# LittleWat/multichannel-semseg-with-uda

Hardware: AMD Instinct MI355X
Metric: RGB-D img/s (6x480x640) MCD train step, drn_d_38 (higher is better)
Workload: dtype f32 (operands split 2-way into scaled fp16, 3 cross terms on the fp16 MFMA pipe, fp32 accumulate)

## Files before the change

### multichannel-semseg-with-uda_amd/csrc/conv_gemm_split.hip

```cpp
#include <cstdlib>
#include <type_traits>

#include "conv_split_params.h"
#include "options.h"

namespace {


template <class P, int WM, int WN, int WAVES_M, int WAVES_N, bool DGRAD, bool PRESPLIT>
__global__ __launch_bounds__(256, 2) void conv_gemm_split_kernel(ConvSplitParams p) {
  constexpr int BM = 32 * WM * WAVES_M;
  constexpr int BN = 32 * WN * WAVES_N;
  constexpr int NT = 256;
  static_assert(WAVES_M * WAVES_N == 4, "4 waves per workgroup");
  constexpr int B_ITEMS = BN * 2 / NT;
  constexpr int NP = P::NP;
  constexpr int NQ = 2 * NP;
  typedef typename P::frag frag;
  constexpr int A_CHUNKS = NQ * BM;
  constexpr int A_ITERS = (A_CHUNKS + NT - 1) / NT;
  constexpr bool A_EXACT = (A_CHUNKS % NT) == 0;
  constexpr bool A_DMA = A_EXACT;
  constexpr int A_ITERS_DMA = ((2 * P::NPU * BM) % NT == 0) ? (2 * P::NPU * BM) / NT : A_ITERS;
  constexpr int A_BYTES = NQ * BM * 16, B_BYTES = NQ * BN * 16;

  constexpr bool B_DMA = PRESPLIT && A_DMA && (B_ITEMS == 1 || (BM == 128 && BN == 256));
  constexpr int NSTAGE = (B_DMA && 3 * (A_BYTES + B_BYTES) <= 80 * 1024) ? 3 : 2;

  __shared__ __attribute__((aligned(16))) unsigned char smem[NSTAGE * (A_BYTES + B_BYTES)];
  unsigned char* As = smem;
  unsigned char* Bs = smem + NSTAGE * A_BYTES;

  const int t = threadIdx.x;
  const int lane = t & 63;
  const int wave = t >> 6;
  const int wm = wave / WAVES_N;
  const int wn = wave % WAVES_N;
  const int l31 = lane & 31, lh = lane >> 5;

  const int m_tiles = p.Mp / BM;
  const bool SUB = DGRAD && p.sub != 0;
  const int n_tiles = SUB ? p.cls_tile0[4] : p.tile_n1;
  const int tile_n0 = SUB ? 0 : p.tile_n0;
  const int per_xcd = (n_tiles - tile_n0 + 7) >> 3;
  const int xcd = blockIdx.x & 7;
  const int slot = blockIdx.x >> 3;
  const int tile_m = slot % m_tiles;
  const int tile_n = tile_n0 + xcd * per_xcd + slot / m_tiles;
  if (tile_n >= n_tiles) return;

  const int bj = t % BN;
  const int bh0 = __builtin_amdgcn_readfirstlane(t / BN);
  const int HWd = p.Hd * p.Wd;
  const int HWs = p.Hs * p.Ws;
  int cls = 0;
  const bool ILV = SUB && p.sub == 2;
  const bool ROW = SUB && p.sub == 3;
  if (SUB) cls = ILV ? (tile_n & 3) : (tile_n >= p.cls_tile0[1]) + (tile_n >= p.cls_tile0[2]) + (tile_n >= p.cls_tile0[3]);
  const int ry = ROW ? cls : cls >> 1, rx = cls & 1;
  const int Hc = SUB ? (p.Hd - ry + 1) >> 1 : p.Hd;
  const int Wc = SUB && !ROW ? (p.Wd - rx + 1) >> 1 : p.Wd;
  const int HWc = Hc * Wc;
  const int Pc = SUB ? p.N * HWc : p.P;
  const int ltile = SUB ? (ILV ? tile_n >> 2 : tile_n - p.cls_tile0[cls]) : tile_n;
  const int pix = ltile * BN + bj;
  const bool pv = pix < Pc;
  int pn = 0, py = 0, px = 0, yc = 0, xc = 0;
  if (pv) {
    pn = pix / HWc;
    const int rem = pix - pn * HWc;
    yc = rem / Wc;
    xc = rem - yc * Wc;
    py = SUB ? 2 * yc + ry : yc;
    px = SUB && !ROW ? 2 * xc + rx : xc;
  }
  unsigned cls_taps = 0;
  if (SUB) {
    for (int q = 0; q < p.KH * p.KW; ++q) {
      const int qy = q / p.KW, qx = q - qy * p.KW;
      if ((((ry + p.pad - qy * p.dil) | (ROW ? 0 : rx + p.pad - qx * p.dil)) & 1) == 0) cls_taps |= 1u << q;
    }
  }
  constexpr unsigned OOB = 0x80000000u;
  constexpr unsigned UNIT = PRESPLIT ? 16u : 4u;
  const __amdgpu_buffer_rsrc_t src_rs = PRESPLIT ? __builtin_amdgcn_make_buffer_rsrc((void*)p.src_cb, 0, p.cb_bytes, 0x00020000)
                                                 : __builtin_amdgcn_make_buffer_rsrc((void*)p.src, 0, p.src_bytes, 0x00020000);
  __amdgpu_buffer_rsrc_t cb_rs[NP];
#pragma unroll
  for (int pc = 0; pc < NP; ++pc)
    cb_rs[pc] = __builtin_amdgcn_make_buffer_rsrc((void*)((const char*)p.src_cb + pc * p.cb_piece_stride), 0, PRESPLIT ? p.cb_bytes : 0, 0x00020000);
  const __amdgpu_buffer_rsrc_t wp_rs = __builtin_amdgcn_make_buffer_rsrc((void*)p.wp, 0, p.wp_bytes, 0x00020000);
  const int C8 = p.Cs >> 3;
  const float inv_src_scale = 1.f / operand_scale<P>(p.src_bound);
  const unsigned pix_base = PRESPLIT ? (unsigned)pn * (unsigned)C8 * (unsigned)HWs : (unsigned)pn * (unsigned)p.Cs * (unsigned)HWs;
  const bool ragged = p.Kp != p.Cs;
  const int taps = p.KH * p.KW;

  int l_tap = 0, l_c0 = 0, l_ky = 0, l_kx = 0, l_kstep = 0;
  unsigned l_voff = OOB;
  auto tap_geom = [&]() {
    bool ok;
    int off;
    if (!DGRAD) {
      const int sy = py * p.stride + l_ky * p.dil - p.pad;
      const int sx = px * p.stride + l_kx * p.dil - p.pad;
      ok = pv && sy >= 0 && sy < p.Hs && sx >= 0 && sx < p.Ws;
      off = sy * p.Ws + sx;
    } else {
      const int ty = py + p.pad - l_ky * p.dil;
      const int tx = px + p.pad - l_kx * p.dil;
      ok = pv && ty >= 0 && tx >= 0;
      int sy = ty, sx = tx;
// ... 112 lines not shown
    const int a_soff = (l_kstep * NQ * p.Mp + tile_m * BM) * 16;
    if (A_DMA) return;
#pragma unroll
    for (int i = 0; i < A_ITERS; ++i) {
      const auto q = __builtin_amdgcn_raw_buffer_load_b128(wp_rs, a_voff[i], a_soff, 0);
      areg[SET][i][0] = __uint_as_float(q[0]);
      areg[SET][i][1] = __uint_as_float(q[1]);
      areg[SET][i][2] = __uint_as_float(q[2]);
      areg[SET][i][3] = __uint_as_float(q[3]);
    }
  };
  auto dma_weights = [&](int buf) {
    const int a_soff = (l_kstep * NQ * p.Mp + tile_m * BM) * 16;
    unsigned char* adst = As + buf * A_BYTES + wave * 64 * 16;
#if defined(__HIP_DEVICE_COMPILE__)
#pragma unroll
    for (int i = 0; i < A_ITERS_DMA; ++i)
      __builtin_amdgcn_raw_ptr_buffer_load_lds(wp_rs, (__attribute__((address_space(3))) void*)(adst + i * NT * 16), 16, a_voff[i], a_soff, 0, 0);
#else
    (void)a_soff;
    (void)adst;
#endif
  };
  auto store_lds = [&](int buf, auto set_c) {
    constexpr int SET = decltype(set_c)::value;
    unsigned char* bdst = Bs + buf * B_BYTES;
#pragma unroll
    for (int it = 0; it < B_ITEMS; ++it) {
      const int h = (B_ITEMS == 1) ? bh0 : it;
      if constexpr (PRESPLIT) {
#pragma unroll
        for (int pc = 0; pc < NP; ++pc) *reinterpret_cast<f32x4*>(bdst + ((pc * 2 + h) * BN + bj) * 16) = bsplit[SET][it][pc];
        continue;
      }
      if constexpr (!PRESPLIT) {
        frag pieces[NP];
        split_frag<P>(breg[SET][it], inv_src_scale, pieces);
#pragma unroll
        for (int pc = 0; pc < NP; ++pc) *reinterpret_cast<frag*>(bdst + ((pc * 2 + h) * BN + bj) * 16) = pieces[pc];
      }
    }
    if (!A_DMA) {
      unsigned char* adst = As + buf * A_BYTES;
#pragma unroll
      for (int i = 0; i < A_ITERS; ++i) {
        const int id = t + i * NT;
        if (A_EXACT || id < A_CHUNKS) *reinterpret_cast<f32x4*>(adst + id * 16) = areg[SET][i];
      }
    }
  };

  f32x16 acc[WM][WN];
#pragma unroll
  for (int i = 0; i < WM; ++i)
#pragma unroll
    for (int j = 0; j < WN; ++j)
#pragma unroll
      for (int r = 0; r < 16; ++r) acc[i][j][r] = 0.f;

  const int nsteps = (SUB ? __builtin_popcount(cls_taps) : taps) * (p.Kp / 16);
  using S0 = std::integral_constant<int, 0>;
  using S1 = std::integral_constant<int, 1>;
  int l_dma_kstep = l_kstep;
  int dma_tap = l_tap, dma_c0 = 0;
  auto dma_b = [&](int buf) {
    const int wave_px = __builtin_amdgcn_readfirstlane(bj - lane);
#pragma unroll
    for (int it = 0; it < B_ITEMS; ++it) {
      const int h = (B_ITEMS == 1) ? bh0 : it;
      const int grp = (l_c0 >> 3) + h;
      unsigned char* bdst = Bs + buf * B_BYTES + (h * BN + wave_px) * 16;
#if defined(__HIP_DEVICE_COMPILE__)
#pragma unroll
      for (int pc = 0; pc < P::NPU; ++pc) {
        const int soff = grp < C8 ? grp * HWs * 16 : 0x7FFFFFFF;
        __builtin_amdgcn_raw_ptr_buffer_load_lds(cb_rs[pc], (__attribute__((address_space(3))) void*)(bdst + pc * 2 * BN * 16), 16, l_voff, soff, 0, 0);
      }
#else
      (void)grp;
      (void)bdst;
#endif
    }
  };
  constexpr int DMA_PER_STEP = A_ITERS_DMA + P::NPU * B_ITEMS;
  if constexpr (B_DMA) {
    if (nsteps > 0) {
      dma_weights(0);
      dma_b(0);
    }
    if (NSTAGE == 3 && nsteps > 1) {
      advance();
      dma_weights(1);
      dma_b(1);
      asm volatile("s_waitcnt vmcnt(%0) lgkmcnt(0)\n\ts_barrier" ::"n"(DMA_PER_STEP) : "memory");
    } else {
      asm volatile("s_waitcnt vmcnt(0) lgkmcnt(0)\n\ts_barrier" ::: "memory");
    }
  } else {
    if (nsteps > 0) {
      if (A_DMA) dma_weights(0);
      load_regs(S0{});
      store_lds(0, S0{});
      if (nsteps > 1) {
        advance();
        load_regs(S1{});
      }
    }
    __syncthreads();
  }

  frag fa[NP][WM], fb[NP][WN];
  auto read_frags = [&](int cur) {
    const unsigned char* a_base = As + cur * A_BYTES + (lh * BM + wm * (32 * WM) + l31) * 16;
    const unsigned char* b_base = Bs + cur * B_BYTES + (lh * BN + wn * (32 * WN) + l31) * 16;
#pragma unroll
    for (int pc = 0; pc < NP; ++pc) {
#pragma unroll
      for (int i = 0; i < WM; ++i) fa[pc][i] = *reinterpret_cast<const frag*>(a_base + (pc * 2 * BM + i * 32) * 16);
#pragma unroll
      for (int j = 0; j < WN; ++j) fb[pc][j] = *reinterpret_cast<const frag*>(b_base + (pc * 2 * BN + j * 32) * 16);
    }
  };
  auto mfma_frags = [&]() {
#if defined(MCD_SETPRIO)
    __builtin_amdgcn_s_setprio(1);
#endif
#if defined(MCD_MFMA_TILE_MAJOR)
#pragma unroll
    for (int i = 0; i < WM; ++i)
#pragma unroll
      for (int j = 0; j < WN; ++j)
#pragma unroll
        for (int tm = 0; tm < P::NTERMS; ++tm) acc[i][j] = P::mfma(fa[P::TA[tm]][i], fb[P::TB[tm]][j], acc[i][j]);
#else
#pragma unroll
    for (int tm = 0; tm < P::NTERMS; ++tm)
#pragma unroll
      for (int i = 0; i < WM; ++i)
#pragma unroll
        for (int j = 0; j < WN; ++j) acc[i][j] = P::mfma(fa[P::TA[tm]][i], fb[P::TB[tm]][j], acc[i][j]);
#endif
#if defined(MCD_SETPRIO)
    __builtin_amdgcn_s_setprio(0);
#endif
  };
  auto mfma_step = [&](int cur) {
    read_frags(cur);
    mfma_frags();
  };
  auto k_step = [&](int s, auto cur_c, auto steady_c) {
    constexpr int CUR = decltype(cur_c)::value;
    constexpr bool STEADY = decltype(steady_c)::value;
    using SAME = std::integral_constant<int, CUR>;
    using OTHER = std::integral_constant<int, CUR ^ 1>;
    if (A_DMA && (STEADY || s + 1 < nsteps)) {
      if (SUB) {
        const unsigned rest = cls_taps & ~((2u << dma_tap) - 1u);
        if (rest) {
          dma_tap = __builtin_ctz(rest);
        } else {
          dma_tap = __builtin_ctz(cls_taps);
          dma_c0 += 16;
        }
        l_dma_kstep = (dma_c0 >> 4) * taps + dma_tap;
      } else {
        ++l_dma_kstep;
// ... 18 lines not shown
    if (STEADY || s + 1 < nsteps) store_lds(CUR ^ 1, OTHER{});
    if constexpr (A_DMA) {
      constexpr int AHEAD = (PRESPLIT ? NP : 8) * B_ITEMS;
      if (STEADY || s + 2 < nsteps)
        asm volatile("s_waitcnt vmcnt(%0) lgkmcnt(0)\n\ts_barrier" ::"n"(AHEAD) : "memory");
      else
        asm volatile("s_waitcnt vmcnt(0) lgkmcnt(0)\n\ts_barrier" ::: "memory");
    } else {
      __syncthreads();
    }
  };
  using YES = std::integral_constant<bool, true>;
  using NO = std::integral_constant<bool, false>;
  if constexpr (B_DMA && NSTAGE == 3) {
    int cur = 0, nxt2 = 2;
    for (int s = 0; s < nsteps; ++s) {
      const bool more2 = s + 2 < nsteps;
#if defined(MCD_ABLATE) && (MCD_ABLATE & 4)
      if (s == 0)
#endif
      read_frags(cur);
      __builtin_amdgcn_sched_barrier(0);
      if (more2) {
        advance();
#if !defined(MCD_ABLATE) || !(MCD_ABLATE & 1)
        dma_weights(nxt2);
#endif
#if defined(MCD_ABLATE) && (MCD_ABLATE & 64)
        if (l_tap == 0) dma_b(nxt2);
#elif !defined(MCD_ABLATE) || !(MCD_ABLATE & 2)
        dma_b(nxt2);
#endif
      }
      __builtin_amdgcn_sched_barrier(0);
#if !defined(MCD_ABLATE) || !(MCD_ABLATE & 8)
      mfma_frags();
#endif
#if defined(MCD_ABLATE) && (MCD_ABLATE & 16)
      asm volatile("s_waitcnt lgkmcnt(0)\n\ts_barrier" ::: "memory");
#elif defined(MCD_ABLATE) && (MCD_ABLATE & 32)
      if (more2)
        asm volatile("s_waitcnt vmcnt(%0) lgkmcnt(0)" ::"n"(DMA_PER_STEP) : "memory");
      else
        asm volatile("s_waitcnt vmcnt(0) lgkmcnt(0)" ::: "memory");
#elif defined(MCD_ABLATE) && (MCD_ABLATE & 128)
      if (s & 1) {
        if (more2)
          asm volatile("s_waitcnt vmcnt(%0) lgkmcnt(0)\n\ts_barrier" ::"n"(DMA_PER_STEP) : "memory");
        else
          asm volatile("s_waitcnt vmcnt(0) lgkmcnt(0)\n\ts_barrier" ::: "memory");
      } else {
        asm volatile("s_waitcnt lgkmcnt(0)" ::: "memory");
      }
#else
      if (more2)
        asm volatile("s_waitcnt vmcnt(%0) lgkmcnt(0)\n\ts_barrier" ::"n"(DMA_PER_STEP) : "memory");
      else
        asm volatile("s_waitcnt vmcnt(0) lgkmcnt(0)\n\ts_barrier" ::: "memory");
#endif
      cur = cur == 2 ? 0 : cur + 1;
      nxt2 = nxt2 == 2 ? 0 : nxt2 + 1;
    }
  } else if constexpr (B_DMA) {
    for (int s = 0; s < nsteps; ++s) {
      const int cur = s & 1;
      if (s + 1 < nsteps) {
        advance();
        dma_weights(cur ^ 1);
        dma_b(cur ^ 1);
      }
      mfma_step(cur);
      asm volatile("s_waitcnt vmcnt(0) lgkmcnt(0)\n\ts_barrier" ::: "memory");
    }
  } else {
    int s = 0;
    for (; s + 3 < nsteps; s += 2) {
      k_step(s, S0{}, YES{});
      k_step(s + 1, S1{}, YES{});
    }
    for (; s < nsteps; s += 2) {
      k_step(s, S0{}, NO{});
      if (s + 1 < nsteps) k_step(s + 1, S1{}, NO{});
    }
  }

  if constexpr (P::SCALED) {
    const float osc = mcd_scale_of_bound(*p.src_bound) * mcd_scale_of_bound(*p.w_bound);
#pragma unroll
    for (int i = 0; i < WM; ++i)
#pragma unroll
      for (int j = 0; j < WN; ++j)
#pragma unroll
        for (int r = 0; r < 16; ++r) acc[i][j][r] *= osc;
  }
  const int m_wave = tile_m * BM + wm * (32 * WM);
  const int p_wave = tile_n * BN + wn * (32 * WN);
  if (!DGRAD && p.bias != nullptr) {
#pragma unroll
    for (int i = 0; i < WM; ++i)
#pragma unroll
      for (int r = 0; r < 16; ++r) {
        const int m = m_wave + i * 32 + (r & 3) + 8 * (r >> 2) + 4 * lh;
        const float bv = (m < p.M) ? p.bias[m] : 0.f;
#pragma unroll
        for (int j = 0; j < WN; ++j) acc[i][j][r] += bv;
      }
  }
  if (!DGRAD && p.ep_scale != nullptr) {
#pragma unroll
    for (int i = 0; i < WM; ++i)
#pragma unroll
      for (int r = 0; r < 16; ++r) {
        const int m = m_wave + i * 32 + (r & 3) + 8 * (r >> 2) + 4 * lh;
        const float sc = (m < p.M) ? p.ep_scale[m] : 0.f;
        const float sh = (m < p.M) ? p.ep_shift[m] : 0.f;
#pragma unroll
        for (int j = 0; j < WN; ++j) acc[i][j][r] = fmaf(acc[i][j][r], sc, sh);
      }
  }
  bool colv[WN];
  size_t dbase[WN];
  size_t ubase[P::HALF_OUT ? WN : 1];
#pragma unroll
  for (int j = 0; j < WN; ++j) {
    const int pp = ltile * BN + wn * (32 * WN) + j * 32 + l31;
    colv[j] = pp < Pc;
    int n = 0, rem = 0;
    if (colv[j]) {
      n = pp / HWc;
      rem = pp - n * HWc;
      if (SUB) {
        const int cy = rem / Wc;
        rem = ROW ? (2 * cy + ry) * p.Wd + (rem - cy * Wc) : (2 * cy + ry) * p.Wd + 2 * (rem - cy * Wc) + rx;
      }
    }
    dbase[j] = (size_t)n * p.M * HWd + rem;
    if constexpr (P::HALF_OUT) ubase[j] = (size_t)n * (p.M >> 3) * HWd + rem;
  }
  bool half_out = false;
  if constexpr (P::HALF_OUT) half_out = p.dst16 != nullptr;
  if constexpr (P::HALF_OUT) {
    if (half_out) {
      float inv_zs = 1.f;
      if (!DGRAD) {
        const float zb = (float)(taps * p.Cs) * (*p.src_bound) * (*p.w_bound);
        inv_zs = 1.f / mcd_scale_of_bound(zb);
        if (blockIdx.x == 0 && t == 0 && p.dst_bound != nullptr) *p.dst_bound = zb;
      }
#pragma unroll
      for (int i = 0; i < WM; ++i)
#pragma unroll
        for (int q = 0; q < 4; ++q) {
          const int m0 = m_wave + i * 32 + 8 * q;
          if (m0 < p.M) {
            const size_t gofs = (size_t)(m0 >> 3) * HWd;
#pragma unroll
            for (int j = 0; j < WN; ++j)
              if (colv[j]) {
                const size_t byte = (ubase[j] + gofs) * 16 + lh * 8;
                float v[4];
#pragma unroll
                for (int k = 0; k < 4; ++k) v[k] = acc[i][j][4 * q + k];
                if (DGRAD) {
                  if (p.ep_res16 != nullptr) {
                    const mcd_bf16x4 add = *reinterpret_cast<const mcd_bf16x4*>((const char*)p.ep_res16 + byte);
#pragma unroll
// ... 190 lines not shown
    __syncthreads();
    if (mode == 0) {
      for (int idx = t; idx < MT * 16 * T; idx += 256) {
        const int mm = idx / (16 * T), col = idx - mm * (16 * T);
        const int kk = col / T;
        tile[mm * row_len + col] = (m0 + mm < M && k0 + kk < K) ? w[((int64_t)(m0 + mm) * Cin + k0) * T + col] : 0.f;
      }
    } else {
      for (int idx = t; idx < 16 * MT * T; idx += 256) {
        const int kk = idx / (MT * T), col = idx - kk * (MT * T);
        const int mm = col / T, tap = col - mm * T;
        tile[mm * row_len + kk * T + tap] = (m0 + mm < M && k0 + kk < K) ? w[((int64_t)(k0 + kk) * Cin + m0) * T + col] : 0.f;
      }
    }
    __syncthreads();
    for (int u = t; u < T * 2 * MT; u += 256) {
      const int mm = u % MT, r = u / MT;
      const int h = r & 1, tap = r >> 1;
      float v[8];
#pragma unroll
      for (int el = 0; el < 8; ++el) v[el] = tile[mm * row_len + (8 * h + el) * T + tap];
      typename P::frag q[NP];
      split_frag<P>(v, inv_scale, q);
      const int64_t base = ((int64_t)chunk * T + tap) * (2 * NP) * (int64_t)Mp * 8;
#pragma unroll
      for (int pc = 0; pc < NP; ++pc) *reinterpret_cast<typename P::frag*>(out + base + ((pc * 2 + h) * (int64_t)Mp + m0 + mm) * 8) = q[pc];
    }
  }
}

int split_check(const mcdseg_conv_desc* d, int math, const char* who, bool operands = true) {
  MCD_REQUIRE(d != nullptr, "%s: null descriptor", who);
  MCD_REQUIRE(mcd_math_known(math), "%s: math must be MCDSEG_MATH_BF16X6, MCDSEG_MATH_F16X3 or MCDSEG_MATH_F16X1 (got %d)", who, math);
  MCD_REQUIRE(d->N > 0 && d->Cin > 0 && d->H > 0 && d->W > 0 && d->Cout > 0, "%s: non-positive dims", who);
  MCD_REQUIRE(d->KH > 0 && d->KW > 0 && d->stride > 0 && d->dil > 0 && d->pad >= 0, "%s: bad kernel geometry", who);
  const int ho = (d->H + 2 * d->pad - d->dil * (d->KH - 1) - 1) / d->stride + 1;
  const int wo = (d->W + 2 * d->pad - d->dil * (d->KW - 1) - 1) / d->stride + 1;
  MCD_REQUIRE(ho == d->Ho && wo == d->Wo, "%s: Ho/Wo (%d,%d) do not match geometry (%d,%d)", who, d->Ho, d->Wo, ho, wo);
  MCD_REQUIRE(!operands || ((int64_t)d->N * d->Cin * d->H * d->W * 4 < (1ll << 31) && (int64_t)d->N * d->Cout * d->Ho * d->Wo * 4 < (1ll << 31)),
              "%s: activation tensor must stay below 2 GiB (32-bit buffer offsets); split the batch", who);
  return 0;
}

int64_t split_image_bytes(int math, int M, int K, int T) {
  return (int64_t)(round_up(K, 16) / 16) * T * 2 * mcd_math_pieces(math) * mcd_mp(M) * 16;
}

int big_tile_min_slots() { return (int)mcd_opt(MCD_OPT_BIGTILE_MIN_SLOTS); }

template <class P, int WM, int WN, int WAVES_M, int WAVES_N, bool DGRAD>
void launch_cfg(const ConvSplitParams& p, int64_t pix0, hipStream_t st) {
  constexpr int BM = 32 * WM * WAVES_M, BN = 32 * WN * WAVES_N;
  ConvSplitParams q = p;
  q.sub = 0;
  int n_tiles = ceil_div(p.P, BN);
  q.tile_n0 = (int)(pix0 / BN);
  q.tile_n1 = n_tiles;
  n_tiles -= q.tile_n0;
  if (DGRAD && p.stride == 2 && p.KH * p.KW <= 32) {
    q.sub = 1;
    int t0 = 0;
    for (int c = 0; c < 4; ++c) {
      q.cls_tile0[c] = t0;
      const int hc = (p.Hd - (c >> 1) + 1) / 2, wc = (p.Wd - (c & 1) + 1) / 2;
      t0 += ceil_div(p.N * hc * wc, BN);
    }
    q.cls_tile0[4] = t0;
    n_tiles = t0;
    const int c0 = q.cls_tile0[1];
    const bool interleave = mcd_opt(MCD_OPT_DGRAD_INTERLEAVE) != 0;
    if (interleave && q.cls_tile0[2] == 2 * c0 && q.cls_tile0[3] == 3 * c0 && t0 == 4 * c0) q.sub = 2;
    const bool row_auto = interleave && p.KH * p.KW == 1 && p.ep_res == nullptr && p.ep_res16 == nullptr;
    if (mcd_opt(MCD_OPT_DGRAD_INTERLEAVE) == 2 || row_auto) {
      q.sub = 3;
      t0 = 0;
      for (int c = 0; c < 2; ++c) {
        q.cls_tile0[c] = t0;
        t0 += ceil_div(p.N * ((p.Hd - c + 1) / 2) * p.Wd, BN);
      }
      q.cls_tile0[2] = q.cls_tile0[3] = q.cls_tile0[4] = t0;
      n_tiles = t0;
    }
  }
  dim3 grid(8 * ceil_div(n_tiles, 8) * (p.Mp / BM));
  if (p.src_cb != nullptr)
    hipLaunchKernelGGL((conv_gemm_split_kernel<P, WM, WN, WAVES_M, WAVES_N, DGRAD, true>), grid, dim3(256), 0, st, q);
  else
    hipLaunchKernelGGL((conv_gemm_split_kernel<P, WM, WN, WAVES_M, WAVES_N, DGRAD, false>), grid, dim3(256), 0, st, q);
}

int wide_tile_min_slots() { return (int)mcd_opt(MCD_OPT_WIDETILE_MIN_SLOTS); }

int tile_config(int M, int64_t P, bool presplit) {
  const int bm = mcd_bm(M), mp = mcd_mp(M);
  if (bm == 128 && presplit && (mp % 256) == 0 && ceil_div64(P, 128) * (mp / 256) >= big_tile_min_slots()) return 4222;
  if (bm == 128 && presplit && ceil_div64(P, 256) * (mp / 128) >= wide_tile_min_slots()) return 4214;
  if (bm == 128) return 2222;
  return bm == 64 ? 2214 : 1214;
}

template <class P, bool DGRAD>
void launch(const ConvSplitParams& p, int64_t pix0, hipStream_t st) {
  switch (tile_config(p.M, p.P, p.src_cb != nullptr)) {
    case 4222: launch_cfg<P, 4, 2, 2, 2, DGRAD>(p, pix0, st); break;
    case 4214: launch_cfg<P, 4, 2, 1, 4, DGRAD>(p, pix0, st); break;
    case 2222: launch_cfg<P, 2, 2, 2, 2, DGRAD>(p, pix0, st); break;
    case 2214: launch_cfg<P, 2, 2, 1, 4, DGRAD>(p, pix0, st); break;
    default: launch_cfg<P, 1, 2, 1, 4, DGRAD>(p, pix0, st); break;
  }
}

}

int64_t mcdseg_internal_conv_pp_pixels(const ConvSplitParams& p, int math, bool dgrad);
int mcdseg_internal_conv_pp_launch(const ConvSplitParams& p, int math, bool dgrad, int64_t pixels, hipStream_t st);
int mcdseg_internal_conv_pp_rest(const ConvSplitParams& p, int math, bool dgrad);
int mcdseg_internal_conv_pp_wide(const ConvSplitParams& p, int math, bool dgrad);
int mcdseg_internal_conv_pp_deep(const ConvSplitParams& p, int math);
int mcdseg_internal_conv_pp_rest_launch(const ConvSplitParams& p, int math, bool dgrad, int64_t pix0, hipStream_t st);

namespace {

template <bool DGRAD>
int launch_math(int math, const ConvSplitParams& p, int part, hipStream_t st) {
  const int64_t pp = mcdseg_internal_conv_pp_pixels(p, math, DGRAD);
  if (pp > 0 && part != 2)
    if (int rc = mcdseg_internal_conv_pp_launch(p, math, DGRAD, pp, st)) return rc;
  if (pp >= p.P || part == 1) return 0;
  if (mcdseg_internal_conv_pp_rest(p, math, DGRAD)) return mcdseg_internal_conv_pp_rest_launch(p, math, DGRAD, pp, st);
  if (math == MCDSEG_MATH_F16X3)
    launch<SplitF16x3, DGRAD>(p, pp, st);
  else if (math == MCDSEG_MATH_F16X1)
    launch<SplitF16x1, DGRAD>(p, pp, st);
  else
    launch<SplitBf16x6, DGRAD>(p, pp, st);
  return 0;
}

}

bool mcdseg_internal_stem_ok(const mcdseg_conv_desc* d);
int64_t mcdseg_internal_stem_stat_rows(const mcdseg_conv_desc* d);
int64_t mcdseg_internal_stem_image_bytes();
int mcdseg_internal_stem_pack(const mcdseg_conv_desc* d, const float* w, void* out, hipStream_t st);
int mcdseg_internal_stem_fprop(const mcdseg_conv_desc* d, const float* x, const void* wp, const float* bias, float* y, float* stats,
                               const float* ep_scale, const float* ep_shift, const float* ep_res, int ep_relu, hipStream_t st);

int mcdseg_internal_thin_window_ok(const mcdseg_conv_desc* d, int dgrad);
int64_t mcdseg_internal_thin_window_stat_rows(const mcdseg_conv_desc* d);
int mcdseg_internal_thin_window_launch(const mcdseg_conv_desc* d, int dgrad, const void* src_cb, const float* src_bound, const void* wp,
                                       int64_t wp_bytes, const float* w_bound, float* dst, float* stats, hipStream_t st);

static int64_t stem_image_offset(const mcdseg_conv_desc* d, int math) {
  return (split_image_bytes(math, d->Cout, d->Cin, d->KH * d->KW) + 255) / 256 * 256;
}

extern "C" int32_t mcdseg_conv_split_direct_ok(const mcdseg_conv_desc* d) { return d != nullptr && mcdseg_internal_stem_ok(d) ? 1 : 0; }

static int64_t stat_rows_of(const mcdseg_conv_desc* d, bool presplit) {
  const int cfg = tile_config(d->Cout, (int64_t)d->N * d->Ho * d->Wo, presplit);
  const int64_t waves_n = cfg % 10, bn = 32 * ((cfg / 100) % 10) * waves_n;
  return ceil_div64((int64_t)d->N * d->Ho * d->Wo, bn) * waves_n;
}

extern "C" int64_t mcdseg_conv_split_stat_rows(const mcdseg_conv_desc* d) {
  if (d == nullptr) return -22;
  if (mcdseg_internal_stem_ok(d)) return mcdseg_internal_stem_stat_rows(d);
  return stat_rows_of(d, false);
}
// ... 88 lines not shown
  if (math == MCDSEG_MATH_F16X3) {
    (void)hipMemsetAsync(bounds, 0, sizeof(float) * (size_t)n, st);
    hipLaunchKernelGGL(absmax_multi_kernel, dim3(48, (unsigned)n), dim3(256), 0, st, ptrs, dims);
    MCD_LAUNCH_CHECK("absmax_multi");
    hipLaunchKernelGGL(pack_weights_multi_kernel<SplitF16x3>, dim3(pack_blocks, 2u * (unsigned)n), dim3(256), 0, st, ptrs, dims);
  } else {
    hipLaunchKernelGGL(pack_weights_multi_kernel<SplitBf16x6>, dim3(pack_blocks, 2u * (unsigned)n), dim3(256), 0, st, ptrs, dims);
  }
  MCD_LAUNCH_CHECK("conv_split_pack_weights_multi");
  return 0;
}

static int split_cb_bytes(const mcdseg_conv_desc* d, int math, int C, int HW, const void* cb, int* piece_bytes, long long* piece_stride) {
  *piece_bytes = 0;
  *piece_stride = 0;
  if (cb == nullptr) return 0;
  MCD_REQUIRE((C % 8) == 0, "conv_split: a pre-split operand needs a channel count divisible by 8 (got %d)", C);
  MCD_REQUIRE(d->Ncb == 0 || d->Ncb >= d->N, "conv_split: Ncb (%d) must be 0 or at least N (%d)", d->Ncb, d->N);
  const int64_t b = (int64_t)d->N * C * HW * 2;
  MCD_REQUIRE(b < (1ll << 31), "conv_split: one piece of the pre-split operand exceeds 2 GiB; split the batch");
  *piece_bytes = (int)b;
  *piece_stride = math == MCDSEG_MATH_F16X1 ? 0 : (long long)(d->Ncb ? d->Ncb : d->N) * C * HW * 2;
  return 0;
}

static int fill_fprop_params(const mcdseg_conv_desc* d, int math, const void* x_cb, ConvSplitParams& p);

static int split_fprop_impl(const mcdseg_conv_desc* d, int math, const float* x, const void* x_cb, const float* x_bound, const void* wp,
                            const float* w_bound, const float* bias, float* y, float* stats, const float* ep_scale,
                            const float* ep_shift, const float* ep_res, int ep_relu, void* stream, int part = 0, void* z16 = nullptr,
                            float* z_bound = nullptr) {
  if (int rc = split_check(d, math, "conv_split_fprop", z16 == nullptr)) return rc;
  MCD_REQUIRE((x || x_cb) && wp && (y || z16), "conv_split_fprop: null pointer");
  if (z16 != nullptr) {
    MCD_REQUIRE(mcdseg_conv_split_half_ok(d, math, 0) && x_cb != nullptr && z_bound != nullptr && bias == nullptr && ep_scale == nullptr,
                "conv_split_fprop_half: the 16-bit output needs f16x1, a pre-split input, channel counts divisible by 8, a bound scalar "
                "to write and no bias / affine epilogue (mcdseg_conv_split_half_ok tells)");
    MCD_REQUIRE((int64_t)d->N * d->Cout * d->Ho * d->Wo * 2 < (1ll << 32), "conv_split_fprop_half: output above 4 GiB; split the batch");
  }
  const bool stem = mcdseg_internal_stem_ok(d);
  const int smath = mcd_storage_math(math);
  const bool stem_window = stem && smath == MCDSEG_MATH_F16X3 && x_cb != nullptr && bias == nullptr && ep_scale == nullptr &&
                           mcdseg_internal_thin_window_ok(d, 0);
  if (part == 1 && (stem || (smath == MCDSEG_MATH_F16X3 && x_cb != nullptr && mcdseg_internal_thin_window_ok(d, 0)))) return 0;
  if (stem && !stem_window) {
    MCD_REQUIRE(x != nullptr, "conv_split_fprop: the stem kernel reads the fp32 input");
    return mcdseg_internal_stem_fprop(d, x, (const char*)wp + stem_image_offset(d, math), bias, y, stats, ep_scale, ep_shift, ep_res,
                                      ep_relu, (hipStream_t)stream);
  }
  MCD_REQUIRE(smath != MCDSEG_MATH_F16X3 || (x_bound && w_bound), "conv_split_fprop: f16x3 needs the operand and weight bound scalars");
  if (smath == MCDSEG_MATH_F16X3 && x_cb != nullptr && mcdseg_internal_thin_window_ok(d, 0)) {
    MCD_REQUIRE(bias == nullptr && ep_scale == nullptr, "conv_split_fprop: the thin-layer window kernel takes no bias / affine epilogue");
    return mcdseg_internal_thin_window_launch(d, 0, x_cb, x_bound, wp, split_image_bytes(math, d->Cout, d->Cin, d->KH * d->KW), w_bound, y,
                                              stats, (hipStream_t)stream);
  }
  ConvSplitParams p;
  if (int rc = fill_fprop_params(d, math, x_cb, p)) return rc;
  p.src_bound = x_bound; p.w_bound = w_bound;
  p.src = x; p.wp = wp; p.bias = bias; p.dst = y; p.stats = stats;
  p.ep_scale = ep_scale; p.ep_shift = ep_shift; p.ep_res = ep_res; p.ep_relu = ep_relu;
  p.dst16 = z16; p.dst_bound = z_bound;
  if (int rc = launch_math<false>(math, p, part, (hipStream_t)stream)) return rc;
  MCD_LAUNCH_CHECK("conv_split_fprop");
  return 0;
}

static int fill_fprop_params(const mcdseg_conv_desc* d, int math, const void* x_cb, ConvSplitParams& p) {
  if (int rc = split_cb_bytes(d, math, d->Cin, d->H * d->W, x_cb, &p.cb_bytes, &p.cb_piece_stride)) return rc;
  p.src_cb = x_cb;
  p.N = d->N;
  p.Cs = d->Cin; p.Hs = d->H; p.Ws = d->W;
  p.M = d->Cout; p.Hd = d->Ho; p.Wd = d->Wo;
  p.Mp = mcd_mp(d->Cout);
  p.Kp = round_up(d->Cin, 16);
  p.KH = d->KH; p.KW = d->KW; p.stride = d->stride; p.pad = d->pad; p.dil = d->dil;
  p.P = d->N * d->Ho * d->Wo;
  p.src_bytes = (int)((int64_t)d->N * d->Cin * d->H * d->W * 4);
  const int64_t wb = split_image_bytes(math, d->Cout, d->Cin, d->KH * d->KW);
  MCD_REQUIRE(wb < (1ll << 31), "conv_split_fprop: packed weights exceed 2 GiB");
  p.wp_bytes = (int)wb;
  p.sub = 0; p.tile_n0 = 0; p.tile_n1 = 0;
  p.ep_res_lds = 0; p.ep_res_bytes = 0;
  p.dst16 = nullptr; p.dst_bound = nullptr; p.ep_res16 = nullptr;
  return 0;
}

extern "C" int mcdseg_conv_split_fprop(const mcdseg_conv_desc* d, int32_t math, const float* x, const void* x_cb, const float* x_bound,
                                       const void* wp_fprop, const float* w_bound, const float* bias, float* y, float* stat_partials,
                                       void* stream) {
  return split_fprop_impl(d, math, x, x_cb, x_bound, wp_fprop, w_bound, bias, y, stat_partials, nullptr, nullptr, nullptr, 0, stream);
}

extern "C" int mcdseg_conv_split_fprop_affine(const mcdseg_conv_desc* d, int32_t math, const float* x, const void* x_cb,
                                              const float* x_bound, const void* wp_fprop, const float* w_bound, const float* scale,
                                              const float* shift, const float* residual, int32_t relu, float* y, void* stream) {
  MCD_REQUIRE(scale && shift, "conv_split_fprop_affine: null scale/shift");
  return split_fprop_impl(d, math, x, x_cb, x_bound, wp_fprop, w_bound, nullptr, y, nullptr, scale, shift, residual, relu, stream);
}

static int fill_dgrad_params(const mcdseg_conv_desc* d, int math, const void* dy_cb, ConvSplitParams& p) {
  if (int rc = split_cb_bytes(d, math, d->Cout, d->Ho * d->Wo, dy_cb, &p.cb_bytes, &p.cb_piece_stride)) return rc;
  p.src_cb = dy_cb;
  p.N = d->N;
  p.Cs = d->Cout; p.Hs = d->Ho; p.Ws = d->Wo;
  p.M = d->Cin; p.Hd = d->H; p.Wd = d->W;
  p.Mp = mcd_mp(d->Cin);
  p.Kp = round_up(d->Cout, 16);
  p.KH = d->KH; p.KW = d->KW; p.stride = d->stride; p.pad = d->pad; p.dil = d->dil;
  p.P = d->N * d->H * d->W;
  p.src_bytes = (int)((int64_t)d->N * d->Cout * d->Ho * d->Wo * 4);
  const int64_t wb = split_image_bytes(math, d->Cin, d->Cout, d->KH * d->KW);
  MCD_REQUIRE(wb < (1ll << 31), "conv_split_dgrad: packed weights exceed 2 GiB");
  p.wp_bytes = (int)wb;
  p.sub = 0; p.tile_n0 = 0; p.tile_n1 = 0;
  p.ep_res_lds = 0; p.ep_res_bytes = 0;
  p.dst16 = nullptr; p.dst_bound = nullptr; p.ep_res16 = nullptr;
  return 0;
}

static int split_dgrad_impl(const mcdseg_conv_desc* d, int32_t math, const float* dy, const void* dy_cb, const float* dy_bound,
                            const void* wp_dgrad, const float* w_bound, float* dx, void* stream, int part, const float* addend = nullptr,
                            void* dx16 = nullptr, const void* addend16 = nullptr) {
  if (int rc = split_check(d, math, "conv_split_dgrad", dx16 == nullptr)) return rc;
  MCD_REQUIRE((dy || dy_cb) && wp_dgrad && (dx || dx16), "conv_split_dgrad: null pointer");
  if (dx16 != nullptr) {
    MCD_REQUIRE(mcdseg_conv_split_half_ok(d, math, 1) && dy_cb != nullptr && addend == nullptr,
                "conv_split_dgrad_half: the 16-bit output needs f16x1, a pre-split gradient and channel counts divisible by 8 "
                "(mcdseg_conv_split_half_ok tells)");
    MCD_REQUIRE((int64_t)d->N * d->Cin * d->H * d->W * 2 < (1ll << 32), "conv_split_dgrad_half: output above 4 GiB; split the batch");
  }
  const int smath = mcd_storage_math(math);
  MCD_REQUIRE(smath != MCDSEG_MATH_F16X3 || (dy_bound && w_bound), "conv_split_dgrad: f16x3 needs the operand and weight bound scalars");
  MCD_REQUIRE(addend == nullptr || !(smath == MCDSEG_MATH_F16X3 && dy_cb != nullptr && mcdseg_internal_thin_window_ok(d, 1)),
              "conv_split_dgrad_add: the thin-layer window kernel takes no addend (mcdseg_conv_split_window_ok tells)");
  if (smath == MCDSEG_MATH_F16X3 && dy_cb != nullptr && mcdseg_internal_thin_window_ok(d, 1))
    return part == 1 ? 0
                     : mcdseg_internal_thin_window_launch(d, 1, dy_cb, dy_bound, wp_dgrad, split_image_bytes(math, d->Cin, d->Cout, d->KH * d->KW),
                                                          w_bound, dx, nullptr, (hipStream_t)stream);
  ConvSplitParams p;
  if (int rc = fill_dgrad_params(d, math, dy_cb, p)) return rc;
  p.src_bound = dy_bound; p.w_bound = w_bound;
  p.src = dy; p.wp = wp_dgrad; p.bias = nullptr; p.dst = dx; p.stats = nullptr;
  p.ep_scale = nullptr; p.ep_shift = nullptr; p.ep_res = addend; p.ep_relu = 0;
  p.dst16 = dx16; p.ep_res16 = addend16;
  if (addend != nullptr) {
    const bool stage = mcd_opt(MCD_OPT_DGRAD_ADD_LDS) != 0;
    const int64_t bytes = (int64_t)d->N * d->Cin * d->H * d->W * 4;
    p.ep_res_lds = stage && ((d->H * d->W) & 3) == 0 && (reinterpret_cast<uintptr_t>(addend) & 15) == 0 && bytes < (1ll << 32) ? 1 : 0;
    p.ep_res_bytes = (unsigned)(bytes < (1ll << 32) ? bytes : 0);
  }
  if (int rc = launch_math<true>(math, p, part, (hipStream_t)stream)) return rc;
  MCD_LAUNCH_CHECK("conv_split_dgrad");
  return 0;
}

extern "C" int mcdseg_conv_split_dgrad(const mcdseg_conv_desc* d, int32_t math, const float* dy, const void* dy_cb, const float* dy_bound,
                                       const void* wp_dgrad, const float* w_bound, float* dx, void* stream) {
  return split_dgrad_impl(d, math, dy, dy_cb, dy_bound, wp_dgrad, w_bound, dx, stream, 0);
}

extern "C" int mcdseg_conv_split_dgrad_add(const mcdseg_conv_desc* d, int32_t math, const float* dy, const void* dy_cb, const float* dy_bound,
                                           const void* wp_dgrad, const float* w_bound, const float* addend, float* dx, int32_t part,
                                           void* stream) {
  MCD_REQUIRE(part >= 0 && part <= 2, "conv_split_dgrad_add: part must be 0 (whole), 1 (ping-pong tiles) or 2 (the rest)");
  MCD_REQUIRE(addend != nullptr && addend != dx, "conv_split_dgrad_add: the addend is a tensor of its own");
  return split_dgrad_impl(d, math, dy, dy_cb, dy_bound, wp_dgrad, w_bound, dx, stream, part, addend);
}

extern "C" int64_t mcdseg_conv_split_parts(const mcdseg_conv_desc* d, int32_t math, int32_t presplit, int32_t dgrad) {
  if (d == nullptr || !mcd_math_known(math) || !presplit) return 0;
  const int smath = mcd_storage_math(math);
  if (smath == MCDSEG_MATH_F16X3 && mcdseg_internal_thin_window_ok(d, dgrad ? 1 : 0)) return 0;
  if (!dgrad && mcdseg_internal_stem_ok(d)) return 0;
  ConvSplitParams p;
  if (dgrad ? fill_dgrad_params(d, math, d, p) : fill_fprop_params(d, math, d, p)) return 0;
  return mcdseg_internal_conv_pp_pixels(p, math, dgrad != 0);
}

extern "C" int32_t mcdseg_conv_split_rest_pingpong(const mcdseg_conv_desc* d, int32_t math, int32_t presplit, int32_t dgrad) {
  if (d == nullptr || !mcd_math_known(math) || !presplit) return 0;
  const int smath = mcd_storage_math(math);
  if (smath == MCDSEG_MATH_F16X3 && mcdseg_internal_thin_window_ok(d, dgrad ? 1 : 0)) return 0;
  if (!dgrad && mcdseg_internal_stem_ok(d)) return 0;
  ConvSplitParams p;
  if (dgrad ? fill_dgrad_params(d, math, d, p) : fill_fprop_params(d, math, d, p)) return 0;
  return mcdseg_internal_conv_pp_rest(p, math, dgrad != 0);
}

extern "C" int32_t mcdseg_conv_split_wide_pingpong(const mcdseg_conv_desc* d, int32_t math, int32_t presplit, int32_t dgrad) {
  if (d == nullptr || !mcd_math_known(math) || !presplit) return 0;
  const int smath = mcd_storage_math(math);
  if (smath == MCDSEG_MATH_F16X3 && mcdseg_internal_thin_window_ok(d, dgrad ? 1 : 0)) return 0;
  if (!dgrad && mcdseg_internal_stem_ok(d)) return 0;
  ConvSplitParams p;
  if (dgrad ? fill_dgrad_params(d, math, d, p) : fill_fprop_params(d, math, d, p)) return 0;
  return mcdseg_internal_conv_pp_wide(p, math, dgrad != 0);
}

extern "C" int mcdseg_conv_split_fprop_part(const mcdseg_conv_desc* d, int32_t math, const float* x, const void* x_cb, const float* x_bound,
// ... 43 lines not shown
```

### multichannel-semseg-with-uda_amd/csrc/conv_split_params.h

```cpp
#pragma once
#include "split.h"

struct ConvSplitParams {
  const float* src;
  const void* src_cb;
  const void* wp;
  const float* src_bound;
  const float* w_bound;
  const float* bias;
  float* dst;
  float* stats;
  const float* ep_scale;
  const float* ep_shift;
  const float* ep_res;
  int ep_relu;
  int N;
  int Cs, Hs, Ws;
  int M, Hd, Wd;
  int Mp, Kp;
  int KH, KW, stride, pad, dil;
  int P;
  int src_bytes, wp_bytes, cb_bytes;
  long long cb_piece_stride;
  int sub;
  int cls_tile0[5];
  int tile_n0, tile_n1;
  int ep_res_lds;
  unsigned ep_res_bytes;
  void* dst16;
  float* dst_bound;
  const void* ep_res16;
  int skip_dead;
};

typedef _Float16 mcd_f16x4 __attribute__((ext_vector_type(4)));
typedef __bf16 mcd_bf16x4 __attribute__((ext_vector_type(4)));
```

### multichannel-semseg-with-uda_amd/csrc/options.h

```cpp
#pragma once
#include <stdint.h>

#define MCD_OPTIONS(X)                                                                                                       \
  X(BN_STATS_ONE, 1024)                     \
  X(BN_REVERSE, 1)                              \
  X(BN_V4, 1)                                         \
  X(BIGTILE_MIN_SLOTS, 1024)                               \
  X(WIDETILE_MIN_SLOTS, 1024)                                                                 \
  X(DGRAD_INTERLEAVE, 1)       \
  X(DGRAD_ADD_LDS, 1)                   \
  X(PACK_BLOCKS, 192)                               \
  X(PP_MIN_ROUNDS, 2)          \
  X(PP_CUS, 0)                 \
  X(PINGPONG, 3)               \
  X(PP_WIDE_FILL, 80)                               \
  X(PP_WIDE128, 1)                                                                                \
  X(PP_DEEP, 1)                \
  X(SKIP_DEAD_TAPS, 1)         \
  X(THIN_WINDOW, 1)                                                           \
  X(WGRAD_WGS, 1024)                                  \
  X(WGRAD_THIN_TR, 1)                                                               \
  X(WGRAD_TR64, 1)                                                    \
  X(WGRAD_BIG, 1)                                                                       \
  X(WGRAD_PP_CUS, 0)                          \
  X(WGRAD_PP, 2)                                          \
  X(WGRAD_PP3, 1)                                                                 \
  X(WGRAD_PP_DEEP, 1)          \
  X(UP8_LOSS_DMA, 1)                                  \
  X(UP8_BAND_ROWS, -1)

enum McdOpt {
#define X(name, def) MCD_OPT_##name,
  MCD_OPTIONS(X)
#undef X
      MCD_OPT_COUNT
};

int64_t mcd_opt(McdOpt which);
```

Before: 83.24.

## Add LDS halo-window path for 3x3 stride-1 convs on the 64x256 f16x3 tile

Adds a windowed implicit-GEMM path for 3x3, stride-1, pad-1 convolutions on the BM=64/BN=256 f16x3 presplit configuration. For each 16-channel chunk it stages a halo window of input rows into LDS once, then runs all nine taps by shifting LDS offsets, instead of re-gathering the B operand for every tap. Weights are loaded straight from global memory into registers with double buffering. The window extends into dynamic LDS beyond the static staging buffer, which may reduce occupancy, and the path is enabled by default through a new option.

```diff
diff --git a/multichannel-semseg-with-uda_amd/csrc/conv_gemm_split.hip b/multichannel-semseg-with-uda_amd/csrc/conv_gemm_split.hip
--- a/multichannel-semseg-with-uda_amd/csrc/conv_gemm_split.hip
+++ b/multichannel-semseg-with-uda_amd/csrc/conv_gemm_split.hip
@@ -27,7 +27,12 @@
   constexpr bool B_DMA = PRESPLIT && A_DMA && (B_ITEMS == 1 || (BM == 128 && BN == 256));
   constexpr int NSTAGE = (B_DMA && 3 * (A_BYTES + B_BYTES) <= 80 * 1024) ? 3 : 2;
 
-  __shared__ __attribute__((aligned(16))) unsigned char smem[NSTAGE * (A_BYTES + B_BYTES)];
+  constexpr bool WINDOW = PRESPLIT && std::is_same<P, SplitF16x3>::value && WM == 2 && WN == 2 && WAVES_M == 1 && WAVES_N == 4;
+  constexpr int STAGE_BYTES = NSTAGE * (A_BYTES + B_BYTES);
+  static_assert(!WINDOW || STAGE_BYTES == MCD_WINDOW64_STATIC, "the host sizes the window launch's dynamic LDS by this");
+
+  __shared__ __attribute__((aligned(16))) unsigned char smem[STAGE_BYTES];
+  extern __shared__ __attribute__((aligned(16))) unsigned char win_dyn[];
   unsigned char* As = smem;
   unsigned char* Bs = smem + NSTAGE * A_BYTES;
 
@@ -306,6 +311,95 @@
 #endif
     }
   };
+  bool windowed = false;
+  if constexpr (WINDOW) windowed = p.window != 0 && mcd_lds_addr(win_dyn) == mcd_lds_addr(smem) + (unsigned)STAGE_BYTES;
+  if (windowed) {
+    if constexpr (WINDOW) {
+      const int W = p.Ws, Wc = W + 2, ncell = p.window;
+      const int tile_pix = tile_n * BN;
+      const int n_img = tile_pix / HWd, rem0 = tile_pix - n_img * HWd;
+      const int y0 = rem0 / W, y1 = (rem0 + BN - 1) / W;
+      const int wv = __builtin_amdgcn_readfirstlane(wave);
+      const __amdgpu_buffer_rsrc_t win_rs = (wv >> 1) ? cb_rs[1] : cb_rs[0];
+      const int wh = wv & 1;
+      const int r_first = lane / Wc, c_first = lane - r_first * Wc;
+      const int dq = 64 / Wc, dr = 64 - dq * Wc;
+      const int iters = ncell >> 6;
+      auto stage = [&](int chunk) {
+        const int soff = ((n_img * C8 + 2 * chunk + wh) * HWs) * 16;
+        unsigned char* dst = smem + wv * ncell * 16;
+        int r = r_first, cx = c_first;
+        for (int it = 0; it < iters; ++it) {
+          const int y = y0 - 1 + r, x = cx - 1;
+          const bool ok = r < p.window_rows && y >= 0 && y < p.Hs && y <= y1 + 1 && x >= 0 && x < W;
+          const unsigned voff = ok ? (unsigned)(y * W + x) * 16u : OOB;
+#if defined(__HIP_DEVICE_COMPILE__)
+          __builtin_amdgcn_raw_ptr_buffer_load_lds(win_rs, (__attribute__((address_space(3))) void*)(dst + it * 64 * 16), 16, voff, soff, 0, 0);
+#else
+          (void)voff; (void)soff; (void)dst;
+#endif
+          cx += dr;
+          r += dq;
+          if (cx >= Wc) {
+            cx -= Wc;
+            ++r;
+          }
+        }
+      };
+      unsigned ub[WN];
+#pragma unroll
+      for (int j = 0; j < WN; ++j) {
+        const int rem = rem0 + wn * (32 * WN) + j * 32 + l31;
+        const int y = rem / W, x = rem - y * W;
+        ub[j] = (unsigned)(lh * ncell + (y - y0) * Wc + x) * 16u;
+      }
+      const unsigned a_v = ((unsigned)lh * (unsigned)p.Mp + (unsigned)(wm * (32 * WM) + l31)) * 16u;
+      auto load_a = [&](frag (&a)[NP][WM], int kstep) {
+        const int base = (kstep * NQ * p.Mp + tile_m * BM) * 16;
+#pragma unroll
+        for (int pc = 0; pc < NP; ++pc)
+#pragma unroll
+          for (int i = 0; i < WM; ++i)
+            a[pc][i] = __builtin_bit_cast(frag, __builtin_amdgcn_raw_buffer_load_b128(wp_rs, a_v, base + (pc * 2 * p.Mp + i * 32) * 16, 0));
+      };
+      auto win_step = [&](const frag (&a)[NP][WM], int tap) {
+        const int ky = tap / 3, kx = tap - 3 * ky;
+        const unsigned shift = (unsigned)(DGRAD ? (2 - ky) * Wc + (2 - kx) : ky * Wc + kx) * 16u;
+        frag b[NP][WN];
+#pragma unroll
+        for (int pc = 0; pc < NP; ++pc)
+#pragma unroll
+          for (int j = 0; j < WN; ++j) b[pc][j] = *reinterpret_cast<const frag*>(smem + (unsigned)(pc * 2 * ncell) * 16u + ub[j] + shift);
+#pragma unroll
+        for (int tm = 0; tm < P::NTERMS; ++tm)
+#pragma unroll
+          for (int i = 0; i < WM; ++i)
+#pragma unroll
+            for (int j = 0; j < WN; ++j) acc[i][j] = P::mfma(a[P::TA[tm]][i], b[P::TB[tm]][j], acc[i][j]);
+      };
+      const int chunks = p.Kp / 16;
+      frag a0[NP][WM], a1[NP][WM];
+      load_a(a0, 0);
+      for (int ch = 0; ch < chunks; ++ch) {
+        __syncthreads();
+        stage(ch);
+        __syncthreads();
+#pragma unroll
+        for (int tap = 0; tap < 9; ++tap) {
+          if (tap < 8 || ch + 1 < chunks) load_a((tap & 1) ? a0 : a1, ch * 9 + tap + 1);
+          __builtin_amdgcn_sched_barrier(0);
+          win_step((tap & 1) ? a1 : a0, tap);
+          __builtin_amdgcn_sched_barrier(0);
+        }
+        if (ch + 1 < chunks) {
+#pragma unroll
+          for (int pc = 0; pc < NP; ++pc)
+#pragma unroll
+            for (int i = 0; i < WM; ++i) a0[pc][i] = a1[pc][i];
+        }
+      }
+    }
+  } else {
   constexpr int DMA_PER_STEP = A_ITERS_DMA + P::NPU * B_ITEMS;
   if constexpr (B_DMA) {
     if (nsteps > 0) {
@@ -490,6 +584,7 @@
       k_step(s, S0{}, NO{});
       if (s + 1 < nsteps) k_step(s + 1, S1{}, NO{});
     }
+  }
   }
 
   if constexpr (P::SCALED) {
@@ -846,9 +941,21 @@
       n_tiles = t0;
     }
   }
+  q.window = q.window_rows = 0;
+  if (std::is_same<P, SplitF16x3>::value && BM == 64 && BN == 256 && p.src_cb != nullptr && mcd_opt(MCD_OPT_WINDOW64) != 0 && p.KH == 3 &&
+      p.KW == 3 && p.stride == 1 && p.dil == 1 && p.pad == 1 && p.Hs == p.Hd && p.Ws == p.Wd && (p.Cs % 16) == 0 && p.Kp == p.Cs &&
+      ((p.Hd * p.Wd) % BN) == 0) {
+    const int rows = (2 * p.Wd + BN - 2) / p.Wd + 2;
+    const int cells = round_up(rows * (p.Ws + 2), 64);
+    if (4 * cells * 16 <= MCD_WINDOW64_BYTES) {
+      q.window = cells;
+      q.window_rows = rows;
+    }
+  }
+  const unsigned win_dyn = q.window != 0 && 4 * q.window * 16 > MCD_WINDOW64_STATIC ? 4 * q.window * 16 - MCD_WINDOW64_STATIC : 0;
   dim3 grid(8 * ceil_div(n_tiles, 8) * (p.Mp / BM));
   if (p.src_cb != nullptr)
-    hipLaunchKernelGGL((conv_gemm_split_kernel<P, WM, WN, WAVES_M, WAVES_N, DGRAD, true>), grid, dim3(256), 0, st, q);
+    hipLaunchKernelGGL((conv_gemm_split_kernel<P, WM, WN, WAVES_M, WAVES_N, DGRAD, true>), grid, dim3(256), win_dyn, st, q);
   else
     hipLaunchKernelGGL((conv_gemm_split_kernel<P, WM, WN, WAVES_M, WAVES_N, DGRAD, false>), grid, dim3(256), 0, st, q);
 }
@@ -1103,6 +1210,7 @@
   p.sub = 0; p.tile_n0 = 0; p.tile_n1 = 0;
   p.ep_res_lds = 0; p.ep_res_bytes = 0;
   p.dst16 = nullptr; p.dst_bound = nullptr; p.ep_res16 = nullptr;
+  p.skip_dead = 0; p.window = 0; p.window_rows = 0;
   return 0;
 }
 
@@ -1136,6 +1244,7 @@
   p.sub = 0; p.tile_n0 = 0; p.tile_n1 = 0;
   p.ep_res_lds = 0; p.ep_res_bytes = 0;
   p.dst16 = nullptr; p.dst_bound = nullptr; p.ep_res16 = nullptr;
+  p.skip_dead = 0; p.window = 0; p.window_rows = 0;
   return 0;
 }
 
diff --git a/multichannel-semseg-with-uda_amd/csrc/conv_split_params.h b/multichannel-semseg-with-uda_amd/csrc/conv_split_params.h
--- a/multichannel-semseg-with-uda_amd/csrc/conv_split_params.h
+++ b/multichannel-semseg-with-uda_amd/csrc/conv_split_params.h
@@ -31,7 +31,11 @@
   float* dst_bound;
   const void* ep_res16;
   int skip_dead;
+  int window, window_rows;
 };
+
+constexpr int MCD_WINDOW64_BYTES = 53248;
+constexpr int MCD_WINDOW64_STATIC = 40960;
 
 typedef _Float16 mcd_f16x4 __attribute__((ext_vector_type(4)));
 typedef __bf16 mcd_bf16x4 __attribute__((ext_vector_type(4)));
diff --git a/multichannel-semseg-with-uda_amd/csrc/options.h b/multichannel-semseg-with-uda_amd/csrc/options.h
--- a/multichannel-semseg-with-uda_amd/csrc/options.h
+++ b/multichannel-semseg-with-uda_amd/csrc/options.h
@@ -18,6 +18,7 @@
   X(PP_DEEP, 1)                \
   X(SKIP_DEAD_TAPS, 1)         \
   X(THIN_WINDOW, 1)                                                           \
+  X(WINDOW64, 1)               \
   X(WGRAD_WGS, 1024)                                  \
   X(WGRAD_THIN_TR, 1)                                                               \
   X(WGRAD_TR64, 1)                                                    \
```

New measurement: 83.24 (median of 2 runs). No clear change (+0.0%).
